# ishine/Test-time-adaptation-ASR-SUTA

Hardware: AMD Instinct MI355X
Metric: adapted utterances/sec (whole node) at 10 SUTA steps, w2v2-base; WER parity (higher is better)
Workload: dtype f32; 1 GPU; wav2vec2-base SUTA 10 steps on 128000-sample (8 s) utterances, 164 utterances per GPU per step, scripts/LS.sh flags; model=wav2vec2-base, global_batch=164, seq_len=399, n_samples=128000, suta_steps=10, parallelism=utterance-sharded x1

## Files before the change

test-time-adaptation-asr-suta_amd/csrc/common.h:

```cpp
#pragma once
#include <hip/hip_runtime.h>
#include <stdint.h>
#include <string>

#define SUTA_WAVE 64

typedef float f32x4 __attribute__((ext_vector_type(4)));
typedef float f32x16 __attribute__((ext_vector_type(16)));

__device__ __forceinline__ float gelu_f(float x) {
    return 0.5f * x * (1.0f + erff(x * 0.70710678118654752f));
}
__device__ __forceinline__ float dgelu_f(float x) {
    const float cdf = 0.5f * (1.0f + erff(x * 0.70710678118654752f));
    const float pdf = 0.39894228040143268f * __expf(-0.5f * x * x);
    return cdf + x * pdf;
}

__device__ __forceinline__ float erfc_t(float z, float t, float ez2) {
    float p = 0.17087277f;
    p = fmaf(p, t, -0.82215223f);
    p = fmaf(p, t, 1.48851587f);
    p = fmaf(p, t, -1.13520398f);
    p = fmaf(p, t, 0.27886807f);
    p = fmaf(p, t, -0.18628806f);
    p = fmaf(p, t, 0.09678418f);
    p = fmaf(p, t, 0.37409196f);
    p = fmaf(p, t, 1.00002368f);
    p = fmaf(p, t, -1.26551223f);
    return t * ez2 * __expf(p);
}
__device__ __forceinline__ float gelu_fast(float x) {
    const float z = fabsf(x) * 0.70710678118654752f;
    const float t = __builtin_amdgcn_rcpf(fmaf(0.5f, z, 1.0f));
    const float erfc = erfc_t(z, t, __expf(-z * z));
    return 0.5f * x * (x >= 0.f ? 2.0f - erfc : erfc);
}
__device__ __forceinline__ float dgelu_fast(float x) {
    const float z = fabsf(x) * 0.70710678118654752f;
    const float t = __builtin_amdgcn_rcpf(fmaf(0.5f, z, 1.0f));
    const float e = __expf(-z * z);
    const float erfc = erfc_t(z, t, e);
    const float cdf = 0.5f * (x >= 0.f ? 2.0f - erfc : erfc);
    return cdf + x * (0.39894228040143268f * e);
}

struct SutaSwitches {
    int latched;
    int fast_gelu;
    int flash_fwd_plane;
    int flash_bwd_plane;
    int flash_bf16_img;
    int conv_planes;
    int pre_bf16;
    int conv_z_bf16;
    int dy_planes;
    int conv_dx_planes;
    int fused_conv_ln;
    int flash_fwd_nw;
    int hbx;
    int splitk;
    int hbx_form;
    int ln_rpw;
    int hbx_dbg;
    int fused_delta;
    int hbx_t;
    int hbp_conv;
    int hbt4;
    int epi_fast;
    int loss_wide;
    int f32p;
    int sdpl_wide;
};
void suta_latch_switches();
void set_max_lds_once(const void* fn, size_t bytes, const char* name);
const SutaSwitches& suta_switches();

typedef float f32x2v __attribute__((ext_vector_type(2)));
__device__ __forceinline__ f32x2v phi_as2(f32x2v x, f32x2v& q) {
    const f32x2v z = __builtin_elementwise_abs(x) * 0.70710678118654752f;
    f32x2v p = z * 0.0000430638f + 0.0002765672f;
    p = p * z + 0.0001520143f;
    p = p * z + 0.0092705272f;
    p = p * z + 0.0422820123f;
    p = p * z + 0.0705230784f;
    p = p * z + 1.0f;
    p = p * p;
    p = p * p;
    p = p * p;
    p = p * p;
    q = f32x2v{__builtin_amdgcn_rcpf(p.x), __builtin_amdgcn_rcpf(p.y)};
    const f32x2v h = 0.5f * q;
    return f32x2v{x.x >= 0.f ? 1.0f - h.x : h.x, x.y >= 0.f ? 1.0f - h.y : h.y};
}
__device__ __forceinline__ f32x2v gelu2_bf16ep(f32x2v x) {
    f32x2v q;
    return x * phi_as2(x, q);
}
__device__ __forceinline__ f32x2v dgelu2_bf16ep(f32x2v x) {
    f32x2v q;
    const f32x2v cdf = phi_as2(x, q);
    const f32x2v a = x * x * (-0.5f * 1.4426950408889634f);
    const f32x2v e = f32x2v{__builtin_amdgcn_exp2f(a.x), __builtin_amdgcn_exp2f(a.y)};
    return cdf + (x * 0.39894228040143268f) * e;
}

__device__ __forceinline__ float wave_sum(float v) {
#pragma unroll
    for (int o = 32; o > 0; o >>= 1) v += __shfl_xor(v, o, 64);
    return v;
}
__device__ __forceinline__ double wave_sum_d(double v) {
#pragma unroll
    for (int o = 32; o > 0; o >>= 1) v += __shfl_xor(v, o, 64);
    return v;
}
__device__ __forceinline__ float wave_max(float v) {
#pragma unroll
    for (int o = 32; o > 0; o >>= 1) v = fmaxf(v, __shfl_xor(v, o, 64));
    return v;
}

enum {
    EPI_BIAS = 1,
    EPI_GELU = 2,
    EPI_RESID = 4,
    EPI_STORE_PRE = 8,
    EPI_DGELU = 16,
    EPI_ACCUM = 32,
    EPI_SMBWD = 64,
    EPI_ROWMASK = 128,
    EPI_DELTA = 256,
};

struct GemmParams {
    const float* A;
    const float* B;
    float* C;
    int M, N, K;
    long lda, ldb, ldc;
    int Z, zdiv;
    long sA0, sA1, sB0, sB1, sC0, sC1;
    int ta, tb;
    int segK, pad, Mvalid;
    int segB;
    long sBseg;
    const float* bias;
    long sBias0, sBias1;
    const float* R;
    long ldr, sR0, sR1;
    const float* aux;
    long ldaux, sAux0, sAux1;
    float* C2;
    long ldc2, sC20, sC21;
    const float* rowv;
    long sRow0, sRow1;
    const int* zrows;
    const int* zmvalid;
    float alpha;
    int epi;
    int splits, kchunk;
    float* ws;
    int va, vb;
    int mode;
    int order;
    const void* Ab;
    const void* Bb;
    long ldab, ldbb;
    void* Cb;
    long ldcb;
    long sCb1;
    int off32;
    int preb;
    int fgelu;
    const float* dlt_o;
    long ldo;
    float* delta;
    int dT, dNH;
};

void gemm_init(GemmParams& p);
bool gemm_hbx_t_selected(const GemmParams& p);
void gemm_launch(GemmParams p, hipStream_t st, float* ws, long ws_floats);
void gemm_set_variant(int tile, int nbuf);
void gemm_set_mode(int mode);
bool gemm_run_hb_class(const GemmParams& p, dim3 grid, hipStream_t st);
void launch_to_bf16(const float* src, long lds, long rows, int K, void* dst, hipStream_t st);
void launch_transpose_bf16(const float* src, long zs, int Z, int K, int N, void* dst, hipStream_t st,
                          void* dstn = nullptr);
int gemm_get_mode();
void gemm_census_enable(bool on);
std::string gemm_census_text();
bool gemm_census_is_on();
void gemm_census_time(const std::string& shape, double ms);
```

test-time-adaptation-asr-suta_amd/csrc/gemm.hip:

```cpp
#include "gemm_kernels.h"
#include <algorithm>
#include <cstdio>
#include <cstdlib>
#include <atomic>
#include <map>
#include <mutex>
#include <stdexcept>
#include <string>

namespace {

bool aligned16(const void* q) { return (reinterpret_cast<uintptr_t>(q) & 15) == 0; }

int g_force_tile = -1;
int g_nbuf = 3;
int g_mode = 0;

}

void gemm_set_variant(int tile, int nbuf) {
    g_force_tile = tile;
    g_nbuf = nbuf;
}

static std::mutex g_census_mu;
static std::map<std::string, long> g_census;
static std::atomic<bool> g_census_on{false};
static std::map<std::string, std::pair<double, long>> g_census_ms;

void gemm_census_enable(bool on) {
    std::lock_guard<std::mutex> lk(g_census_mu);
    g_census_on = on;
    g_census.clear();
    g_census_ms.clear();
}

bool gemm_census_is_on() { return g_census_on; }

void gemm_census_time(const std::string& shape, double ms) {
    std::lock_guard<std::mutex> lk(g_census_mu);
    auto& e = g_census_ms[shape];
    e.first += ms;
    e.second += 1;
}

std::string gemm_census_text() {
    std::lock_guard<std::mutex> lk(g_census_mu);
    std::string out;
    for (const auto& kv : g_census) out += kv.first + " " + std::to_string(kv.second) + "\n";
    for (const auto& kv : g_census_ms)
        out += "ms|" + kv.first + "|n=" + std::to_string(kv.second.second) + " " +
               std::to_string((long)(kv.second.first * 1000.0)) + "\n";
    return out;
}

static void census(const char* kernel, int BM, int BN, const GemmParams& p, int splits) {
    if (!g_census_on) return;
    char key[160], gkey[160], ekey[96];
    snprintf(key, sizeof key, "%s %dx%d z=%ld split=%d %s%s%s", kernel, BM, BN, (long)p.Z, splits, p.ta ? "T" : "N",
             p.tb ? "T" : "N", p.segK > 0 ? (p.segB ? " conv-seg" : " conv") : "");
    snprintf(gkey, sizeof gkey, "grid %s %dx%d gx=%d gy=%d z=%ld split=%d", kernel, BM, BN, (p.N + BN - 1) / BN,
             (p.M + BM - 1) / BM, (long)p.Z, splits);
    snprintf(ekey, sizeof ekey, "epi %s %dx%d %d", kernel, BM, BN, p.epi);
    std::lock_guard<std::mutex> lk(g_census_mu);
    ++g_census[key];
    ++g_census[gkey];
    ++g_census[ekey];
}

void gemm_set_mode(int mode) { g_mode = mode; }
int gemm_get_mode() { return g_mode; }

void gemm_init(GemmParams& p) {
    p = GemmParams{};
    p.Z = 1;
    p.zdiv = 1;
    p.alpha = 1.f;
    p.splits = 1;
    p.mode = g_mode;
}

static int choose_tile(long M, long N, long Z, long K, int mode) {
    struct Cand {
        int bm, bn;
        double eff;
    };
    static const Cand glds[4] = {{128, 128, 1.0}, {128, 64, 0.93}, {64, 128, 0.92}, {64, 64, 0.85}};
    static const Cand x6[4] = {{128, 128, 1.0}, {128, 64, 0.9}, {64, 128, 0.9}, {64, 64, 0.75}};
    const Cand* cands = mode == 0 ? glds : x6;
    int best = 0;
    double bt = 1e300;
    for (int c = 0; c < 4; ++c) {
        const long tiles = ((M + cands[c].bm - 1) / cands[c].bm) * ((N + cands[c].bn - 1) / cands[c].bn) * Z;
        const double area = (double)cands[c].bm * cands[c].bn;
        const double t = std::max((double)tiles, 256.0) * area / cands[c].eff;
        if (t < bt * 0.999) {
            bt = t;
            best = c;
        }
    }
    (void)K;
    return best;
}

static int choose_tile_bf16(long M, long N, long Z, bool big) {
    struct Cand {
        int id, bm, bn;
        double eff;
    };
    static const Cand c[5] = {{0, 128, 128, 1.0}, {4, 256, 128, 1.12}, {1, 128, 64, 0.85}, {2, 64, 128, 0.85},
                              {3, 64, 64, 0.6}};
    int best = 0;
    double bt = 1e300;
    for (int i = 0; i < 5; ++i) {
        if (c[i].id == 4 && !big) continue;
        const long tiles = ((M + c[i].bm - 1) / c[i].bm) * ((N + c[i].bn - 1) / c[i].bn) * Z;
        const double t = (double)((tiles + 511) / 512) * c[i].bm * c[i].bn / c[i].eff;
        if (t < bt * 0.999) {
            bt = t;
            best = c[i].id;
        }
    }
    return best;
}

static int choose_tile_hb(long M, long N, long Z) {
// ... 191 lines not shown
```

test-time-adaptation-asr-suta_amd/csrc/ops.h:

```cpp
#pragma once
#include "common.h"

void launch_wave_normalize(const float* x, float* y, int B, long N, const int* lens, hipStream_t st);

void launch_conv0(const float* x, long N, const float* W, const float* bias, long wstride, float* z, int B, int L0,
                  int C, int K, int S, hipStream_t st, void* zb = nullptr);

void launch_front_gn_fwd(const float* x, long N, const float* W, const float* bias, long wstride, int B, int L0, int C,
                         int K, int S, const float* g, const float* beta, float* mean, float* rstd, float* a,
                         double* dpart, const int* L0s, hipStream_t st);
void launch_front_gn_bwd(const float* x, long N, const float* W, const float* bias, long wstride, int B, int L0, int C,
                         int K, int S, const float* g, const float* beta, const float* mean, const float* rstd,
                         float* da, float* dgamma, float* dbeta, float* dW, long gstride, double* dpart, float* fpart,
                         const int* L0s, hipStream_t st);

void launch_layernorm_fwd(const float* x, const float* g, const float* beta, long pstride, int rows_per_utt,
                          float* y, float* xhat, float* rstd, int rows, int D, float eps, int gelu_out,
                          hipStream_t st, void* yb = nullptr, float* mean = nullptr, const void* xb = nullptr);
void launch_layernorm_bwd(const float* dy, const float* xhat, const float* rstd, const float* g, const float* beta,
                          long pstride, int rows_per_utt, int B, int D, int gelu_in, const float* post_aux,
                          const float* resid, float* dx, float* dgamma, float* dbeta, long gstride, float* part,
                          hipStream_t st, void* dxb = nullptr, const float* x = nullptr, const float* mean = nullptr,
                          const void* dyb = nullptr);

long layernorm_bwd_conv_part_floats(int B, int rows_per_utt, int D, int ktaps);
bool launch_layernorm_bwd_conv(const float* dy, const float* rstd, const float* g, const float* beta, long pstride,
                               int rows_per_utt, int B, int D, float* dx, float* dgamma, float* dbeta, float* dbias,
                               float* dw, long gstride, float* part, hipStream_t st, const float* x, const float* mean,
                               const float* xw, long xws, int xs, int ktaps, void* dxb = nullptr, int bf16_in = 0);
void launch_colsum(const float* x, int B, int rows, int C, float* out, long ostride, float* part, hipStream_t st);

struct AdapterW {
    const float *w1, *w1t, *w2, *w2t, *b1, *b2;
    int A, NA, Hp;
};
void launch_adapter_fwd(const float* x, const float* g, const float* beta, long pstride, int rows_per_utt, int B, int H,
                        const AdapterW& w, float eps, float* out, float* mean, float* rstd, hipStream_t st);
int adapter_padded_width(int A);
long adapter_part_floats(int B, int rows_per_utt, int H);
void launch_adapter_bwd(const float* x, const float* dout, const float* mean, const float* rstd, const float* g,
                        const float* beta, long pstride, int rows_per_utt, int B, int H, const AdapterW& w,
                        const int* tlen, float* dx, float* dgamma, float* dbeta, long gstride, float* part,
                        hipStream_t st, void* dxb = nullptr);

bool flash_dh_ok(int dh);
long flash_dq_scratch_floats(int B, int T, int NH, int dh);
bool flash_fwd_reads_plane(bool bf16, const void* qkvb, int H, int dh);
bool flash_bwd_reads_planes(bool bf16, const void* qkvb, const void* dctxb, int H, int dh);
bool launch_flash_fwd(const float* qkv, float* ctx, float* lse, int B, int T, int NH, int H, int dh, float scale,
                      const int* tlen, bool bf16, hipStream_t st, void* ctxb = nullptr, const void* qkvb = nullptr);
bool launch_flash_bwd(const float* qkv, const float* dctx, const float* lse, const float* delta, float* dqkv,
                      float* dqp, int B, int T, int NH, int H, int dh, float scale, const int* tlen, bool bf16,
                      hipStream_t st, void* dqkvb = nullptr, const void* qkvb = nullptr,
                      const void* dctxb = nullptr);
bool flash_wide_dh(int dh);
long flash_wide_dq_scratch_floats(int B, int T, int NH, int dh);
bool launch_flash_wide_fwd(const float* qkv, float* ctx, float* lse, int B, int T, int NH, int H, int dh, float scale,
                           const int* tlen, bool bf16, hipStream_t st, void* ctxb);
bool launch_flash_wide_bwd(const float* qkv, const float* dctx, const float* lse, const float* delta, float* dqkv,
                           float* dqp, int B, int T, int NH, int H, int dh, float scale, const int* tlen, bool bf16,
                           hipStream_t st, void* dqkvb);
bool launch_posconv(bool fwd, const float* x, const float* W, const float* bias, const float* R, float* C, float* C2,
                    int B, int T, int H, int G, int K, int pad, const int* tlen, hipStream_t st);
bool launch_posconv_bf16(bool fwd, const float* x, const void* Wt, const float* bias, const float* R, float* C,
                         float* C2, int B, int T, int H, int G, int K, int pad, const int* tlen, hipStream_t st);
void launch_softmax_rows(float* s, long nrows, int T, long ld, const int* tlen, long rows_per_utt, hipStream_t st);

void launch_attn_delta(const float* dO, const float* O, float* delta, int B, int T, int NH, int dh, hipStream_t st);

void launch_dgelu_mul(const float* g, const float* z, float* out, long n, hipStream_t st);

struct LossHP {
    float temp, em_coef, div_coef;
    int reweight, non_blank;
};
#define SUTA_MAX_VOCAB 1024
size_t suta_loss_scratch_floats(int B, long T, int V);
void launch_suta_loss(const float* logits, int B, int T, int V, LossHP hp, const int* tlen, float* dlogits, float* loss,
                      float* scratch, hipStream_t st);

enum { SDPL_KIND_NORMAL = 0, SDPL_KIND_DROP = 1, SDPL_KIND_SPACE = 2, SDPL_KIND_FAIL = 3 };
enum { SDPL_FLAG_LOOKUP = 1, SDPL_FLAG_INFEASIBLE = 2 };
struct SdplTable {
    const int* off;
    const int* ids;
    const int* kind;
    int space_id;
};
long sdpl_scratch_floats(int T, int V);
void launch_sdpl_loss(const float* logits, int B, int T, int V, float pl_coef, const int* tlen, float* dlogits,
                      float* loss, float* scratch, int* err, const SdplTable* tab, hipStream_t st);

void launch_argmax(const float* logits, long rows, int V, int* ids, hipStream_t st);

struct AdamRun {
    long start, len;
    int k;
};
#define SUTA_MAX_RUNS 32
#define ADAM_TAB 52
struct AdamArgs {
    int nruns;
    AdamRun runs[SUTA_MAX_RUNS];
    int blk0[SUTA_MAX_RUNS];
    float beta1, beta2, omb1, omb2, eps, lr_wd;
    int sgd;
    float step_size[5][5];
    float bc2_sqrt[5][5];
    const float* tab;
    const int* step;
};
void launch_broadcast(float* dst, const float* src, long n, int B, hipStream_t st);
void launch_step_advance(int* step, hipStream_t st);
void launch_adam(float* P, const float* G, float* M, float* V, long pstride, int B, const AdamArgs& a,
                 hipStream_t st);
```

test-time-adaptation-asr-suta_amd/csrc/ops.hip:

```cpp
#include "ops.h"
#include <algorithm>
#include <map>
#include <mutex>
#include <stdexcept>
#include <string>

namespace {

inline int cdiv(long a, long b) { return (int)((a + b - 1) / b); }

template <typename T>
__device__ __forceinline__ T block_sum(T v, T* red) {
    const int lane = threadIdx.x & 63, w = threadIdx.x >> 6;
#pragma unroll
    for (int o = 32; o > 0; o >>= 1) v += __shfl_xor(v, o, 64);
    __syncthreads();
    if (lane == 0) red[w] = v;
    __syncthreads();
    T s = red[0] + red[1] + red[2] + red[3];
    __syncthreads();
    return s;
}

__global__ __launch_bounds__(256) void wave_normalize_kernel(const float* __restrict__ x, float* __restrict__ y,
                                                             long N, const int* __restrict__ lens) {
    __shared__ double red[4];
    const float* xb = x + (long)blockIdx.x * N;
    float* yb = y + (long)blockIdx.x * N;
    const long n = lens ? lens[blockIdx.x] : N;
    double s = 0.0;
    for (long i = threadIdx.x; i < n; i += 256) s += xb[i];
    s = block_sum(s, red);
    const double mean = s / (double)n;
    double q = 0.0;
    for (long i = threadIdx.x; i < n; i += 256) {
        const double d = (double)xb[i] - mean;
        q += d * d;
    }
    q = block_sum(q, red);
    const float meanf = (float)mean;
    const float denom = (float)sqrt(q / (double)n + 1e-7);
    for (long i = threadIdx.x; i < N; i += 256) yb[i] = i < n ? (xb[i] - meanf) / denom : 0.f;
}

constexpr int C0_ROWS = 32;
__global__ __launch_bounds__(256) void conv0_kernel(const float* __restrict__ x, long N, const float* __restrict__ W,
                                                    const float* __restrict__ bias, long wstride,
                                                    float* __restrict__ z, int L0, int C, int K, int S) {
    __shared__ float xs[C0_ROWS * 16 + 16];
    const int b = blockIdx.y;
    const int t0 = blockIdx.x * C0_ROWS;
    const float* xb = x + (long)b * N;
    const float* Wb = W + (long)b * wstride;
    const float* bb = bias ? bias + (long)b * wstride : nullptr;
    const int nx = (C0_ROWS - 1) * S + K;
    for (int i = threadIdx.x; i < nx; i += 256) {
        const long gi = (long)t0 * S + i;
        xs[i] = gi < N ? xb[gi] : 0.f;
    }
    __syncthreads();
    const int rows = min(C0_ROWS, L0 - t0);
    float* zb = z + ((long)b * L0 + t0) * C;
    for (int c = threadIdx.x; c < C; c += 256) {
        float w[16];
#pragma unroll
        for (int k = 0; k < 16; ++k) w[k] = k < K ? Wb[(long)k * C + c] : 0.f;
        const float bv = bb ? bb[c] : 0.f;
        for (int r = 0; r < rows; ++r) {
            float acc = 0.f;
            for (int k = 0; k < K; ++k) acc = fmaf(xs[r * S + k], w[k], acc);
            zb[(long)r * C + c] = acc + bv;
        }
    }
}

typedef __bf16 lnbf16x4 __attribute__((ext_vector_type(4)));
__device__ __forceinline__ f32x4 load_bf16x4(const __bf16* src) {
    const lnbf16x4 b = *reinterpret_cast<const lnbf16x4*>(src);
    return f32x4{(float)b[0], (float)b[1], (float)b[2], (float)b[3]};
}
__device__ __forceinline__ void store_bf16x4(__bf16* dst, f32x4 v) {
    lnbf16x4 b;
#pragma unroll
    for (int e = 0; e < 4; ++e) b[e] = (__bf16)v[e];
    *reinterpret_cast<lnbf16x4*>(dst) = b;
}

constexpr int C0V_ROWS = 64;
// ... 716 lines not shown
    const int u = (L / ntile) % nutt;
    const int gi = L / (ntile * nutt);
    const int t0 = tile * WROWS;
    const int tl = tlen ? tlen[u] : T;
    const int w = threadIdx.x >> 6, lane = threadIdx.x & 63;
    const int r = lane & 15, g = lane >> 4;
    const float* xb = x + (long)u * T * H + gi * CG;
    const float* wg = W + (long)gi * K * CG * CG;

    const int nwin = (WROWS + K - 1) * (CG / 4);
    for (int it = threadIdx.x; it < nwin; it += NT) {
        const int row = it / (CG / 4), c4 = (it % (CG / 4)) * 4;
        const int t = t0 - pad + row;
        f32x4 v = {0.f, 0.f, 0.f, 0.f};
        if (t >= 0 && t < tl) v = *reinterpret_cast<const f32x4*>(xb + (long)t * H + c4);
        *reinterpret_cast<f32x4*>(win + row * XS + c4) = v;
    }
    f32x4 st[LPT];
    auto load_chunk = [&](int c) {
        const float* src = wg + (long)c * CHT * CG * CG;
#pragma unroll
        for (int n = 0; n < LPT; ++n) {
            const int it = threadIdx.x + n * NT;
            st[n] = it < CHUNK4 ? *reinterpret_cast<const f32x4*>(src + it * 4) : f32x4{0.f, 0.f, 0.f, 0.f};
        }
    };
    auto store_chunk = [&](int buf) {
        float* dst = wbuf + buf * (CHT * CG * WS);
#pragma unroll
        for (int n = 0; n < LPT; ++n) {
            const int it = threadIdx.x + n * NT;
            if (it < CHUNK4) {
                const int row = (it * 4) / CG, col = (it * 4) % CG;
                *reinterpret_cast<f32x4*>(dst + row * WS + col) = st[n];
            }
        }
    };
    f32x4 acc[NC];
#pragma unroll
    for (int nf = 0; nf < NC; ++nf) acc[nf] = f32x4{0.f, 0.f, 0.f, 0.f};
    const int nch = K / CHT;
    load_chunk(0);
    store_chunk(0);
    __syncthreads();
    const float* arow = win + (16 * w + r) * XS + g;
    for (int c = 0; c < nch; ++c) {
        if (c + 1 < nch) load_chunk(c + 1);
        const float* wb = wbuf + (c & 1) * (CHT * CG * WS) + g * WS + r;
#pragma unroll
        for (int qq = 0; qq < CHT; ++qq) {
            const float* ap = arow + (c * CHT + qq) * XS;
            const float* bp = wb + qq * CG * WS;
#pragma unroll
            for (int j = 0; j < CG / 4; ++j) {
                const float a = ap[4 * j];
                float b[NC];
#pragma unroll
                for (int nf = 0; nf < NC; ++nf) b[nf] = bp[4 * j * WS + 16 * nf];
#pragma unroll
                for (int nf = 0; nf < NC; ++nf) acc[nf] = __builtin_amdgcn_mfma_f32_16x16x4f32(a, b[nf], acc[nf], 0, 0, 0);
            }
        }
        if (c + 1 < nch) store_chunk((c + 1) & 1);
        __syncthreads();
    }
#pragma unroll
    for (int i = 0; i < 4; ++i) {
        const int t = t0 + 16 * w + 4 * g + i;
        if (t >= T) continue;
        const long o = ((long)u * T + t) * H + gi * CG;
#pragma unroll
        for (int nf = 0; nf < NC; ++nf) {
            const int co = 16 * nf + r;
            float v;
            if (FWD) {
                v = acc[nf][i] * 1.0f + bias[gi * CG + co];
                C2[o + co] = v;
                v = gelu_f(v) + R[o + co];
            } else {
                v = acc[nf][i] + R[o + co];
                if (tlen && t >= tl) v = 0.f;
            }
            C[o + co] = v;
        }
    }
}

constexpr int PCB_CHT = 4;
constexpr int PCB_RS = 72;
template <int WB, bool FWD>
__global__ __launch_bounds__(WB * 64, 1) void posconv_bf16_kernel(const float* __restrict__ x,
                                                                  const __bf16* __restrict__ Wt,
                                                                  const float* __restrict__ bias,
                                                                  const float* __restrict__ R, float* __restrict__ C,
                                                                  float* __restrict__ C2, int T, int H, int G, int K,
                                                                  int pad, const int* __restrict__ tlen, int ntile,
                                                                  int nutt) {
    constexpr int CG = 64, NT = WB * 64, WROWS = 32 * WB;
    constexpr int CHUNK = PCB_CHT * CG * CG / 8;
    constexpr int LPT = (CHUNK + NT - 1) / NT;
    extern __shared__ __attribute__((aligned(16))) __bf16 pcb_smem[];
    __bf16* win = pcb_smem;
    __bf16* wbuf = pcb_smem + (WROWS + K - 1) * PCB_RS;
    typedef __bf16 b8 __attribute__((ext_vector_type(8)));
    typedef __bf16 b4 __attribute__((ext_vector_type(4)));

    const int nb = gridDim.x;
    int L = blockIdx.x;
    if ((nb & 7) == 0) L = (L & 7) * (nb >> 3) + (L >> 3);
    const int tile = L % ntile;
    const int u = (L / ntile) % nutt;
    const int gi = L / (ntile * nutt);
    const int t0 = tile * WROWS;
    const int tl = tlen ? tlen[u] : T;
    const int w = threadIdx.x >> 6, lane = threadIdx.x & 63, l32 = lane & 31, h = lane >> 5;
    const float* xb = x + (long)u * T * H + gi * CG;
    const __bf16* wg = Wt + (long)gi * K * CG * CG;

    const int nwin = (WROWS + K - 1) * (CG / 4);
    for (int it = threadIdx.x; it < nwin; it += NT) {
        const int row = it / (CG / 4), c4 = (it % (CG / 4)) * 4;
        const int t = t0 - pad + row;
        f32x4 v = {0.f, 0.f, 0.f, 0.f};
        if (t >= 0 && t < tl) v = *reinterpret_cast<const f32x4*>(xb + (long)t * H + c4);
        b4 o;
#pragma unroll
        for (int e = 0; e < 4; ++e) o[e] = (__bf16)v[e];
        *reinterpret_cast<b4*>(win + row * PCB_RS + c4) = o;
    }
    b8 st[LPT];
    auto load_chunk = [&](int c) {
        const b8* src = reinterpret_cast<const b8*>(wg + (long)c * PCB_CHT * CG * CG);
#pragma unroll
        for (int n = 0; n < LPT; ++n) {
            const int it = threadIdx.x + n * NT;
            if (it < CHUNK) st[n] = src[it];
        }
    };
    auto store_chunk = [&](int buf) {
        __bf16* dst = wbuf + buf * (PCB_CHT * CG * PCB_RS);
#pragma unroll
        for (int n = 0; n < LPT; ++n) {
            const int it = threadIdx.x + n * NT;
            if (it < CHUNK) *reinterpret_cast<b8*>(dst + (it >> 3) * PCB_RS + (it & 7) * 8) = st[n];
        }
    };
    f32x16 acc[2];
#pragma unroll
    for (int nf = 0; nf < 2; ++nf)
#pragma unroll
        for (int v = 0; v < 16; ++v) acc[nf][v] = 0.f;
    const int nch = K / PCB_CHT;
    load_chunk(0);
    store_chunk(0);
    __syncthreads();
    const __bf16* arow = win + (32 * w + l32) * PCB_RS + 8 * h;
    for (int c = 0; c < nch; ++c) {
        if (c + 1 < nch) load_chunk(c + 1);
        const __bf16* wb = wbuf + (c & 1) * (PCB_CHT * CG * PCB_RS) + l32 * PCB_RS + 8 * h;
#pragma unroll
        for (int qq = 0; qq < PCB_CHT; ++qq) {
            const __bf16* ap = arow + (c * PCB_CHT + qq) * PCB_RS;
            const __bf16* bp = wb + qq * CG * PCB_RS;
#pragma unroll
            for (int kc = 0; kc < CG / 16; ++kc) {
                const b8 a = *reinterpret_cast<const b8*>(ap + 16 * kc);
// ... 886 lines not shown
            else                                                                                                 \
                hipLaunchKernelGGL((layernorm_bwd_conv_kernel<2, true, KT_, DB_, XB_>), grid, dim3(256), 0, st, dy,   \
                                   rstd, g, beta, pstride, rows_per_utt, dx, part, nchunk, crows, x, mean, xw, xws, \
                                   xs, reinterpret_cast<__bf16*>(dxb));                                          \
        } while (0)
        if (ktaps == 10) {
            if (dyb && xb) LBCB(10, true, true);
            else if (xb) LBCB(10, false, true);
            else return false;
        } else {
            if (dyb && xb) LBCB(0, true, true);
            else if (xb) LBCB(0, false, true);
            else return false;
        }
#undef LBCB
        const int nvec = 3 + ktaps;
        hipLaunchKernelGGL(chunk_reduce_conv, dim3(cdiv(D, 256), B, nvec), dim3(256), 0, st, part, nchunk, nvec, D,
                           dgamma, dbeta, dbias, dw, gstride);
        return true;
    }
#define LBC(GV_, KT_)                                                                                         \
    hipLaunchKernelGGL((layernorm_bwd_conv_kernel<2, GV_, KT_>), grid, dim3(256), 0, st, dy, rstd, g, beta, pstride, \
                       rows_per_utt, dx, part, nchunk, crows, x, mean, xw, xws, xs, reinterpret_cast<__bf16*>(dxb))
    if (ktaps == 10) {
        if (gv) LBC(true, 10);
        else LBC(false, 10);
    } else {
        if (gv) LBC(true, 0);
        else LBC(false, 0);
    }
#undef LBC
    const int nvec = 3 + ktaps;
    hipLaunchKernelGGL(chunk_reduce_conv, dim3(cdiv(D, 256), B, nvec), dim3(256), 0, st, part, nchunk, nvec, D, dgamma,
                       dbeta, dbias, dw, gstride);
    return true;
}

void launch_colsum(const float* x, int B, int rows, int C, float* out, long ostride, float* part, hipStream_t st) {
    const int nchunk = cdiv(rows, CS_ROWS);
    hipLaunchKernelGGL(colsum_partial, dim3(nchunk, B), dim3(256), 0, st, x, rows, C, part, nchunk);
    hipLaunchKernelGGL(chunk_reduce, dim3(cdiv(C, 256), B), dim3(256), 0, st, part, nchunk, 1, C, out, (float*)nullptr,
                       ostride);
}

void launch_softmax_rows(float* s, long nrows, int T, long ld, const int* tlen, long rows_per_utt, hipStream_t st) {
    dim3 grid((unsigned)((nrows + 3) / 4));
    if (T <= 256) hipLaunchKernelGGL(softmax_rows_kernel<4>, grid, dim3(256), 0, st, s, nrows, T, ld, tlen,
                                    rows_per_utt);
    else if (T <= 512) hipLaunchKernelGGL(softmax_rows_kernel<8>, grid, dim3(256), 0, st, s, nrows, T, ld, tlen,
                                    rows_per_utt);
    else if (T <= 1024) hipLaunchKernelGGL(softmax_rows_kernel<16>, grid, dim3(256), 0, st, s, nrows, T, ld, tlen,
                                    rows_per_utt);
    else hipLaunchKernelGGL(softmax_rows_kernel<32>, grid, dim3(256), 0, st, s, nrows, T, ld, tlen,
                                    rows_per_utt);
}

constexpr int PC_CHT = 2;
#define HIPCHK_OPS(x)                                                                        \
    do {                                                                                     \
        if ((x) != hipSuccess) throw std::runtime_error("hipFuncSetAttribute(posconv) failed"); \
    } while (0)

template <int CG, bool FWD>
static void posconv_go(int WB, dim3 grid, size_t lds, hipStream_t st, const float* x, const float* W,
                       const float* bias, const float* R, float* C, float* C2, int T, int H, int G, int K, int pad,
                       const int* tlen, int ntile, int B) {
#define PC(WB_)                                                                                                   \
    do {                                                                                                          \
        set_max_lds_once(reinterpret_cast<const void*>(&posconv_kernel<CG, WB_, PC_CHT, FWD>), 160 * 1024,       \
                         "posconv_kernel");                                                                       \
        hipLaunchKernelGGL((posconv_kernel<CG, WB_, PC_CHT, FWD>), grid, dim3(WB_ * 64), lds, st, x, W, bias, R, C, \
                           C2, T, H, G, K, pad, tlen, ntile, B);                                                  \
    } while (0)
    switch (WB) {
        case 4: PC(4); break;
        case 5: PC(5); break;
        case 6: PC(6); break;
        case 7: PC(7); break;
        default: PC(8); break;
    }
#undef PC
}

bool launch_posconv(bool fwd, const float* x, const float* W, const float* bias, const float* R, float* C, float* C2,
                    int B, int T, int H, int G, int K, int pad, const int* tlen, hipStream_t st) {
    const int CG = H / G;
    if ((CG != 48 && CG != 64) || K % PC_CHT || H % 4) return false;
    int WB = 8;
    long best = 1L << 40;
    for (int wb = 8; wb >= 4; --wb) {
        const long tiles = (T + 16 * wb - 1) / (16 * wb);
        const long waste = tiles * 16 * wb - T;
        if (waste < best) {
            best = waste;
            WB = wb;
        }
    }
    const int ntile = (T + 16 * WB - 1) / (16 * WB);
    const int XS = CG + 4, WS = (CG % 64 == 0) ? CG + 16 : CG;
    const size_t lds = ((size_t)(16 * WB + K - 1) * XS + 2 * PC_CHT * CG * WS) * sizeof(float);
    if (lds > 160 * 1024) return false;
    const dim3 grid((unsigned)((long)G * B * ntile));
    if (CG == 48) {
        if (fwd) posconv_go<48, true>(WB, grid, lds, st, x, W, bias, R, C, C2, T, H, G, K, pad, tlen, ntile, B);
        else posconv_go<48, false>(WB, grid, lds, st, x, W, bias, R, C, C2, T, H, G, K, pad, tlen, ntile, B);
    } else {
        if (fwd) posconv_go<64, true>(WB, grid, lds, st, x, W, bias, R, C, C2, T, H, G, K, pad, tlen, ntile, B);
        else posconv_go<64, false>(WB, grid, lds, st, x, W, bias, R, C, C2, T, H, G, K, pad, tlen, ntile, B);
    }
    return true;
}

template <bool FWD>
static void posconv_bf16_go(int WB, dim3 grid, size_t lds, hipStream_t st, const float* x, const __bf16* W,
                            const float* bias, const float* R, float* C, float* C2, int T, int H, int G, int K, int pad,
                            const int* tlen, int ntile, int B) {
#define PCB(WB_)                                                                                                  \
    do {                                                                                                          \
        set_max_lds_once(reinterpret_cast<const void*>(&posconv_bf16_kernel<WB_, FWD>), 160 * 1024,              \
                         "posconv_bf16_kernel");                                                                  \
        hipLaunchKernelGGL((posconv_bf16_kernel<WB_, FWD>), grid, dim3(WB_ * 64), lds, st, x, W, bias, R, C, C2, T, \
                           H, G, K, pad, tlen, ntile, B);                                                         \
    } while (0)
    switch (WB) {
        case 4: PCB(4); break;
        case 5: PCB(5); break;
        case 6: PCB(6); break;
        case 7: PCB(7); break;
        default: PCB(8); break;
    }
#undef PCB
}

bool launch_posconv_bf16(bool fwd, const float* x, const void* Wt, const float* bias, const float* R, float* C,
                         float* C2, int B, int T, int H, int G, int K, int pad, const int* tlen, hipStream_t st) {
    if (H / G != 64 || H % G || K % PCB_CHT || !Wt) return false;
    int WB = 8;
    long best = 1L << 40;
    for (int wb = 8; wb >= 4; --wb) {
        const long tiles = (T + 32 * wb - 1) / (32 * wb);
        const long waste = tiles * 32 * wb - T;
        if (waste < best) {
            best = waste;
            WB = wb;
        }
    }
    const int ntile = (T + 32 * WB - 1) / (32 * WB);
    const size_t lds = ((size_t)(32 * WB + K - 1) * PCB_RS + 2 * PCB_CHT * 64 * PCB_RS) * sizeof(__bf16);
    if (lds > 160 * 1024) return false;
    const dim3 grid((unsigned)((long)G * B * ntile));
    const __bf16* W = reinterpret_cast<const __bf16*>(Wt);
    if (fwd) posconv_bf16_go<true>(WB, grid, lds, st, x, W, bias, R, C, C2, T, H, G, K, pad, tlen, ntile, B);
    else posconv_bf16_go<false>(WB, grid, lds, st, x, W, bias, R, C, C2, T, H, G, K, pad, tlen, ntile, B);
    return true;
}

void launch_dgelu_mul(const float* g, const float* z, float* out, long n, hipStream_t st) {
    hipLaunchKernelGGL(dgelu_mul_kernel, dim3(ew_grid(n)), dim3(256), 0, st, g, z, out, n);
}

void launch_suta_loss(const float* logits, int B, int T, int V, LossHP hp, const int* tlen, float* dlogits, float* loss,
                      float* scratch, hipStream_t st) {
    if (V < 1 || V > SUTA_MAX_VOCAB) throw std::runtime_error("suta loss: vocab_size outside [1, 1024]");
    if (V <= 64 && !suta_switches().loss_wide) {
        hipLaunchKernelGGL(suta_loss_kernel, dim3(B), dim3(256), 0, st, logits, T, V, hp, dlogits, loss, scratch, tlen);
        return;
    }
    double* rowd = reinterpret_cast<double*>(scratch);
    double* utt = rowd + (size_t)B * T * LW_ROW;
    double* cls = utt + (size_t)B * LW_UTT;
    const long rows = (long)B * T;
    const dim3 rgrid((unsigned)((rows + 3) / 4));
    const double temp = hp.temp;
    hipLaunchKernelGGL(loss_wide_rows_kernel, rgrid, dim3(256), 0, st, logits, T, V, rows, temp, dlogits, rowd, tlen);
    hipLaunchKernelGGL(loss_wide_utt_kernel, dim3(B), dim3(256), 0, st, T, hp.reweight, rowd, utt, tlen);
    hipLaunchKernelGGL(loss_wide_cols_kernel, dim3((V + 63) / 64, B), dim3(256), 0, st, logits, T, V, temp, rowd, cls,
                       tlen);
    hipLaunchKernelGGL(loss_wide_finish_kernel, dim3(B), dim3(256), 0, st, T, V, hp, cls, utt, loss, tlen);
    hipLaunchKernelGGL(loss_wide_grad_kernel, rgrid, dim3(256), 0, st, logits, T, V, rows, hp, rowd, utt, cls, dlogits,
                       tlen);
}

size_t suta_loss_scratch_floats(int B, long T, int V) {
    const size_t narrow = (size_t)B * T * 66 + 64;
    const size_t wide = 2 * ((size_t)B * T * LW_ROW + (size_t)B * LW_UTT + (size_t)B * V * LW_CLS) + 64;
// ... 14 lines not shown
}

void launch_broadcast(float* dst, const float* src, long n, int B, hipStream_t st) {
    if (n % 4) throw std::runtime_error("broadcast length not a multiple of 4");
    const long n4 = n / 4;
    hipLaunchKernelGGL(broadcast_kernel, dim3((unsigned)((n4 + 255) / 256), B), dim3(256), 0, st,
                       reinterpret_cast<f32x4*>(dst), reinterpret_cast<const f32x4*>(src), n4);
}

__global__ void step_advance_kernel(int* step) { *step += 1; }

void launch_step_advance(int* step, hipStream_t st) {
    hipLaunchKernelGGL(step_advance_kernel, dim3(1), dim3(1), 0, st, step);
}

void launch_adam(float* P, const float* G, float* M, float* V, long pstride, int B, const AdamArgs& a,
                 hipStream_t st) {
    AdamArgs aa = a;
    long nblk = 0;
    for (int r = 0; r < a.nruns; ++r) {
        if (a.runs[r].start % 4) throw std::runtime_error("adam run start not 16-B aligned");
        if (a.runs[r].k < 1 || a.runs[r].k > 5) throw std::runtime_error("adam multiplicity outside [1, 5]");
        aa.blk0[r] = (int)nblk;
        nblk += ((a.runs[r].len + 3) / 4 + 256 * ADAM_GPT - 1) / (256 * ADAM_GPT);
    }
    if (nblk == 0) return;
    if (pstride % 4) throw std::runtime_error("adam slot stride not a multiple of 4");
    hipLaunchKernelGGL(adam_kernel, dim3((unsigned)nblk, B), dim3(256), 0, st, P, G, M, V, pstride, aa);
}

void set_max_lds_once(const void* fn, size_t bytes, const char* name) {
    static std::mutex mu;
    static std::map<const void*, size_t> done;
    std::lock_guard<std::mutex> lk(mu);
    auto it = done.find(fn);
    if (it != done.end() && it->second >= bytes) return;
    if (hipFuncSetAttribute(fn, hipFuncAttributeMaxDynamicSharedMemorySize, (int)bytes) != hipSuccess)
        throw std::runtime_error(std::string("hipFuncSetAttribute(") + name + ") failed");
    done[fn] = bytes;
}

static thread_local SutaSwitches g_switches{};

void suta_latch_switches() {
    auto on = [](const char* name) {
        const char* ev = std::getenv(name);
        return (ev && atoi(ev) == 0) ? 0 : 1;
    };
    SutaSwitches s{};
    s.fast_gelu = on("SUTA_FAST_GELU");
    s.flash_fwd_plane = on("SUTA_FLASH_FWD_PLANE");
    s.flash_bwd_plane = on("SUTA_FLASH_BWD_PLANE");
    s.flash_bf16_img = on("SUTA_FLASH_BF16_IMG");
    s.conv_planes = on("SUTA_CONV_PLANES");
    s.pre_bf16 = on("SUTA_PRE_BF16");
    s.conv_z_bf16 = on("SUTA_CONV_Z_BF16");
    s.dy_planes = on("SUTA_DY_PLANES");
    s.conv_dx_planes = on("SUTA_CONV_DX_PLANES");
    s.fused_conv_ln = on("SUTA_FUSED_CONV_LN");
    const char* hbx = std::getenv("SUTA_HBX");
    s.hbx = hbx ? atoi(hbx) : 1;
    s.splitk = on("SUTA_SPLITK");
    const char* hbxt = std::getenv("SUTA_HBX_T");
    s.hbx_t = hbxt ? std::min(2, std::max(0, atoi(hbxt))) : 2;
    s.fused_delta = on("SUTA_FUSED_DELTA");
    const char* lrpw = std::getenv("SUTA_LN_RPW");
    s.ln_rpw = lrpw ? atoi(lrpw) : 2;
    const char* hform = std::getenv("SUTA_HBX_FORM");
    s.hbx_form = hform ? atoi(hform) : 4;
    const char* ht4 = std::getenv("SUTA_HBT4");
    s.hbt4 = ht4 ? atoi(ht4) : 1;
    const char* hdbg = std::getenv("SUTA_HBX_DBG");
    s.hbx_dbg = hdbg ? atoi(hdbg) : 0;
    const char* fnw = std::getenv("SUTA_FLASH_FWD_NW");
    s.flash_fwd_nw = (fnw && atoi(fnw) == 8) ? 8 : 4;
    s.epi_fast = on("SUTA_EPI_FAST");
    s.hbp_conv = on("SUTA_HBP_CONV");
    const char* lw = std::getenv("SUTA_LOSS_WIDE");
    s.loss_wide = (lw && atoi(lw) != 0) ? 1 : 0;
    const char* f32p = std::getenv("SUTA_F32P");
    s.f32p = f32p ? std::min(2, std::max(0, atoi(f32p))) : 1;
    const char* sw = std::getenv("SUTA_SDPL_WIDE");
    s.sdpl_wide = (sw && atoi(sw) != 0) ? 1 : 0;
    s.latched = 1;
    g_switches = s;
}

const SutaSwitches& suta_switches() {
    if (!g_switches.latched) suta_latch_switches();
    return g_switches;
}

static bool fast_gelu_on() { return suta_switches().fast_gelu != 0; }
template <int MODE, typename... Args>
static void launch_conv0_gn(dim3 grid, hipStream_t st, int K, int S, Args... args) {
    if (K == 10 && S == 5 && fast_gelu_on())
        hipLaunchKernelGGL((conv0_gn_kernel<MODE, 10, 5, true>), grid, dim3(256), 0, st, args...);
    else if (K == 10 && S == 5)
        hipLaunchKernelGGL((conv0_gn_kernel<MODE, 10, 5>), grid, dim3(256), 0, st, args...);
    else
        hipLaunchKernelGGL((conv0_gn_kernel<MODE, 0, 0>), grid, dim3(256), 0, st, args...);
}

void launch_front_gn_fwd(const float* x, long N, const float* W, const float* bias, long wstride, int B, int L0, int C,
                         int K, int S, const float* g, const float* beta, float* mean, float* rstd, float* a,
                         double* dpart, const int* L0s, hipStream_t st) {
    const int nchunk = cdiv(L0, F0_ROWS);
    launch_conv0_gn<0>(dim3(nchunk, B), st, K, S, x, N, W, bias, wstride, L0, C, K, S,
                       (const float*)nullptr, (const float*)nullptr, (const float*)nullptr, (const float*)nullptr,
                       (float*)nullptr, (const float*)nullptr, dpart, (float*)nullptr, nchunk, L0s);
    hipLaunchKernelGGL(col_stats_final, dim3(cdiv(C, 256), B), dim3(256), 0, st, dpart, nchunk, L0, C, 1e-5f, mean,
                       rstd, L0s);
    launch_conv0_gn<1>(dim3(nchunk, B), st, K, S, x, N, W, bias, wstride, L0, C, K, S,
                       mean, rstd, g, beta, a, (const float*)nullptr, (double*)nullptr, (float*)nullptr, nchunk, L0s);
}

void launch_front_gn_bwd(const float* x, long N, const float* W, const float* bias, long wstride, int B, int L0, int C,
                         int K, int S, const float* g, const float* beta, const float* mean, const float* rstd,
                         float* da, float* dgamma, float* dbeta, float* dW, long gstride, double* dpart, float* fpart,
                         const int* L0s, hipStream_t st) {
    const int nchunk = cdiv(L0, F0_ROWS);
    launch_conv0_gn<2>(dim3(nchunk, B), st, K, S, x, N, W, bias, wstride, L0, C, K, S,
                       mean, rstd, g, beta, da, (const float*)nullptr, dpart, (float*)nullptr, nchunk, L0s);
    float* coef = reinterpret_cast<float*>(dpart + (long)B * nchunk * 2 * C);
    hipLaunchKernelGGL(gn_bwd_final, dim3(cdiv(C, 256), B), dim3(256), 0, st, dpart, nchunk, C, dgamma, dbeta, gstride,
                       coef);
    launch_conv0_gn<3>(dim3(nchunk, B), st, K, S, x, N, W, bias, wstride, L0, C, K, S,
                       mean, rstd, g, beta, da, coef, (double*)nullptr, fpart, nchunk, L0s);
    hipLaunchKernelGGL(conv0_dw_reduce, dim3(cdiv((long)K * C, 256), B), dim3(256), 0, st, fpart, nchunk, K * C, dW,
                       gstride);
}

void launch_attn_delta(const float* dO, const float* O, float* delta, int B, int T, int NH, int dh, hipStream_t st) {
    const long items = (long)B * T * NH;
    const long vec = items * (dh / 4);
    const dim3 grid((unsigned)((vec + 255) / 256));
    const f32x4* a = reinterpret_cast<const f32x4*>(dO);
    const f32x4* c = reinterpret_cast<const f32x4*>(O);
    switch (dh) {
        case 16: hipLaunchKernelGGL(attn_delta_kernel<4>, grid, dim3(256), 0, st, a, c, delta, items, T, NH); return;
        case 32: hipLaunchKernelGGL(attn_delta_kernel<8>, grid, dim3(256), 0, st, a, c, delta, items, T, NH); return;
        case 64: hipLaunchKernelGGL(attn_delta_kernel<16>, grid, dim3(256), 0, st, a, c, delta, items, T, NH); return;
        case 128: hipLaunchKernelGGL(attn_delta_kernel<32>, grid, dim3(256), 0, st, a, c, delta, items, T, NH); return;
        default:
            if (dh % 4 == 0 && dh <= 128 && (reinterpret_cast<uintptr_t>(dO) & 15) == 0 &&
                (reinterpret_cast<uintptr_t>(O) & 15) == 0) {
                hipLaunchKernelGGL(attn_delta_pad32_kernel, dim3((unsigned)((items * 32 + 255) / 256)), dim3(256), 0, st,
                                   a, c, delta, items, T, NH, dh / 4);
                return;
            }
            hipLaunchKernelGGL(attn_delta_scalar, dim3((unsigned)((items + 255) / 256)), dim3(256), 0, st, dO, O, delta,
                               items, T, NH, dh);
    }
}
```

Baseline: 39.35 utt/s.

## Add span-based positional conv kernel with cost-model planner choosing tile or span

Adds a new positional-convolution kernel in which each 8-wave block covers a span of many 16-frame fragments, with several fragments per wave. This amortizes staging of the weight chunks across more output frames. A planner header models LDS occupancy, rounds over CUs and MFMA throughput, then picks between the existing tile kernel (any WB 4..8) and span variants. The span path is on by default through an env switch. The risks are reduced occupancy from large LDS windows and a cost model whose constants may not match the real hardware.

```diff
diff --git a/test-time-adaptation-asr-suta_amd/csrc/common.h b/test-time-adaptation-asr-suta_amd/csrc/common.h
--- a/test-time-adaptation-asr-suta_amd/csrc/common.h
+++ b/test-time-adaptation-asr-suta_amd/csrc/common.h
@@ -71,6 +71,8 @@
     int loss_wide;
     int f32p;
     int sdpl_wide;
+    int posconv_span;
+    int posconv_wb;
 };
 void suta_latch_switches();
 void set_max_lds_once(const void* fn, size_t bytes, const char* name);
@@ -193,3 +195,4 @@
 std::string gemm_census_text();
 bool gemm_census_is_on();
 void gemm_census_time(const std::string& shape, double ms);
+void gemm_census_count(const std::string& key);
diff --git a/test-time-adaptation-asr-suta_amd/csrc/gemm.hip b/test-time-adaptation-asr-suta_amd/csrc/gemm.hip
--- a/test-time-adaptation-asr-suta_amd/csrc/gemm.hip
+++ b/test-time-adaptation-asr-suta_amd/csrc/gemm.hip
@@ -42,6 +42,12 @@
     auto& e = g_census_ms[shape];
     e.first += ms;
     e.second += 1;
+}
+
+void gemm_census_count(const std::string& key) {
+    if (!g_census_on) return;
+    std::lock_guard<std::mutex> lk(g_census_mu);
+    ++g_census[key];
 }
 
 std::string gemm_census_text() {
diff --git a/test-time-adaptation-asr-suta_amd/csrc/ops.h b/test-time-adaptation-asr-suta_amd/csrc/ops.h
--- a/test-time-adaptation-asr-suta_amd/csrc/ops.h
+++ b/test-time-adaptation-asr-suta_amd/csrc/ops.h
@@ -1,5 +1,6 @@
 #pragma once
 #include "common.h"
+#include "posconv_plan.h"
 
 void launch_wave_normalize(const float* x, float* y, int B, long N, const int* lens, hipStream_t st);
 
@@ -62,6 +63,7 @@
                            hipStream_t st, void* dqkvb);
 bool launch_posconv(bool fwd, const float* x, const float* W, const float* bias, const float* R, float* C, float* C2,
                     int B, int T, int H, int G, int K, int pad, const int* tlen, hipStream_t st);
+bool posconv_plan_for(int B, int T, int H, int G, int K, PosconvPlan* out);
 bool launch_posconv_bf16(bool fwd, const float* x, const void* Wt, const float* bias, const float* R, float* C,
                          float* C2, int B, int T, int H, int G, int K, int pad, const int* tlen, hipStream_t st);
 void launch_softmax_rows(float* s, long nrows, int T, long ld, const int* tlen, long rows_per_utt, hipStream_t st);
diff --git a/test-time-adaptation-asr-suta_amd/csrc/ops.hip b/test-time-adaptation-asr-suta_amd/csrc/ops.hip
--- a/test-time-adaptation-asr-suta_amd/csrc/ops.hip
+++ b/test-time-adaptation-asr-suta_amd/csrc/ops.hip
@@ -4,6 +4,7 @@
 #include <mutex>
 #include <stdexcept>
 #include <string>
+#include <type_traits>
 
 namespace {
 
@@ -886,6 +887,133 @@
                 if (tlen && t >= tl) v = 0.f;
             }
             C[o + co] = v;
+        }
+    }
+}
+
+template <int CG, int FPW, int CHT, bool FWD>
+__global__ __launch_bounds__(512, 1) void posconv_span_kernel(const float* __restrict__ x,
+                                                              const float* __restrict__ W,
+                                                              const float* __restrict__ bias,
+                                                              const float* __restrict__ R, float* __restrict__ C,
+                                                              float* __restrict__ C2, int T, int H, int G, int K,
+                                                              int pad, const int* __restrict__ tlen, int nspan,
+                                                              int nutt, int F) {
+    constexpr int NW = 8, NT = NW * 64, NC = CG / 16, XS = PcLayout<CG>::XS, WS = PcLayout<CG>::WS;
+    constexpr int CHUNK4 = CHT * CG * CG / 4;
+    constexpr int LPT = (CHUNK4 + NT - 1) / NT;
+    extern __shared__ __attribute__((aligned(16))) float pc_smem[];
+    float* win = pc_smem;
+    float* wbuf = pc_smem + (16 * F + K - 1) * XS;
+
+    const int nb = gridDim.x;
+    int L = blockIdx.x;
+    if ((nb & 7) == 0) L = (L & 7) * (nb >> 3) + (L >> 3);
+    const int span = L % nspan;
+    const int u = (L / nspan) % nutt;
+    const int gi = L / (nspan * nutt);
+    const int nf_here = min(F, (T + 15) / 16 - span * F);
+    const int t0 = span * F * 16;
+    const int tl = tlen ? tlen[u] : T;
+    const int w = threadIdx.x >> 6, lane = threadIdx.x & 63;
+    const int r = lane & 15, g = lane >> 4;
+    const int nown = nf_here > w ? (nf_here - w + NW - 1) / NW : 0;
+    const float* xb = x + (long)u * T * H + gi * CG;
+    const float* wg = W + (long)gi * K * CG * CG;
+
+    const int nwin = (16 * nf_here + K - 1) * (CG / 4);
+    for (int it = threadIdx.x; it < nwin; it += NT) {
+        const int row = it / (CG / 4), c4 = (it % (CG / 4)) * 4;
+        const int t = t0 - pad + row;
+        f32x4 v = {0.f, 0.f, 0.f, 0.f};
+        if (t >= 0 && t < tl) v = *reinterpret_cast<const f32x4*>(xb + (long)t * H + c4);
+        *reinterpret_cast<f32x4*>(win + row * XS + c4) = v;
+    }
+    f32x4 st[LPT];
+    auto load_chunk = [&](int c) {
+        const float* src = wg + (long)c * CHT * CG * CG;
+#pragma unroll
+        for (int n = 0; n < LPT; ++n) {
+            const int it = threadIdx.x + n * NT;
+            st[n] = it < CHUNK4 ? *reinterpret_cast<const f32x4*>(src + it * 4) : f32x4{0.f, 0.f, 0.f, 0.f};
+        }
+    };
+    auto store_chunk = [&](int buf) {
+        float* dst = wbuf + buf * (CHT * CG * WS);
+#pragma unroll
+        for (int n = 0; n < LPT; ++n) {
+            const int it = threadIdx.x + n * NT;
+            if (it < CHUNK4) {
+                const int row = (it * 4) / CG, col = (it * 4) % CG;
+                *reinterpret_cast<f32x4*>(dst + row * WS + col) = st[n];
+            }
+        }
+    };
+    f32x4 acc[FPW][NC];
+#pragma unroll
+    for (int i = 0; i < FPW; ++i)
+#pragma unroll
+        for (int nf = 0; nf < NC; ++nf) acc[i][nf] = f32x4{0.f, 0.f, 0.f, 0.f};
+    const int nch = K / CHT;
+    load_chunk(0);
+    store_chunk(0);
+    __syncthreads();
+    const float* arow = win + (16 * w + r) * XS + g;
+    auto taps = [&](auto n_) {
+        constexpr int N = decltype(n_)::value;
+        for (int c = 0; c < nch; ++c) {
+            if (c + 1 < nch) load_chunk(c + 1);
+            const float* wb = wbuf + (c & 1) * (CHT * CG * WS) + g * WS + r;
+#pragma unroll
+            for (int qq = 0; qq < CHT; ++qq) {
+                const float* ap = arow + (c * CHT + qq) * XS;
+                const float* bp = wb + qq * CG * WS;
+#pragma unroll
+                for (int j = 0; j < CG / 4; ++j) {
+                    float a[N > 0 ? N : 1];
+#pragma unroll
+                    for (int i = 0; i < N; ++i) a[i] = ap[i * (16 * NW * XS) + 4 * j];
+                    float b[NC];
+#pragma unroll
+                    for (int nf = 0; nf < NC; ++nf) b[nf] = bp[4 * j * WS + 16 * nf];
+#pragma unroll
+                    for (int i = 0; i < N; ++i)
+#pragma unroll
+                        for (int nf = 0; nf < NC; ++nf)
+                            acc[i][nf] = __builtin_amdgcn_mfma_f32_16x16x4f32(a[i], b[nf], acc[i][nf], 0, 0, 0);
+                }
+            }
+            if (c + 1 < nch) store_chunk((c + 1) & 1);
+            __syncthreads();
+        }
+    };
+    if (nown >= FPW) taps(std::integral_constant<int, FPW>{});
+    else if (FPW > 3 && nown == 3) taps(std::integral_constant<int, (FPW > 3 ? 3 : 0)>{});
+    else if (FPW > 2 && nown == 2) taps(std::integral_constant<int, (FPW > 2 ? 2 : 0)>{});
+    else if (FPW > 1 && nown == 1) taps(std::integral_constant<int, (FPW > 1 ? 1 : 0)>{});
+    else taps(std::integral_constant<int, 0>{});
+#pragma unroll
+    for (int i = 0; i < FPW; ++i) {
+        if (i >= nown) break;
+#pragma unroll
+        for (int ii = 0; ii < 4; ++ii) {
+            const int t = t0 + 16 * (w + NW * i) + 4 * g + ii;
+            if (t >= T) continue;
+            const long o = ((long)u * T + t) * H + gi * CG;
+#pragma unroll
+            for (int nf = 0; nf < NC; ++nf) {
+                const int co = 16 * nf + r;
+                float v;
+                if (FWD) {
+                    v = acc[i][nf][ii] * 1.0f + bias[gi * CG + co];
+                    C2[o + co] = v;
+                    v = gelu_f(v) + R[o + co];
+                } else {
+                    v = acc[i][nf][ii] + R[o + co];
+                    if (tlen && t >= tl) v = 0.f;
+                }
+                C[o + co] = v;
+            }
         }
     }
 }
@@ -1938,25 +2066,77 @@
 #undef PC
 }
 
+template <int CG, bool FWD>
+static void posconv_span_go(const PosconvPlan& pl, hipStream_t st, const float* x, const float* W, const float* bias,
+                            const float* R, float* C, float* C2, int T, int H, int G, int K, int pad, const int* tlen,
+                            int B) {
+#define PCS(FPW_)                                                                                                  \
+    do {                                                                                                           \
+        set_max_lds_once(reinterpret_cast<const void*>(&posconv_span_kernel<CG, FPW_, PC_CHT, FWD>), PC_LDS_MAX,   \
+                         "posconv_span_kernel");                                                                   \
+        hipLaunchKernelGGL((posconv_span_kernel<CG, FPW_, PC_CHT, FWD>), dim3((unsigned)pl.grid), dim3(pl.threads), \
+                           pl.lds, st, x, W, bias, R, C, C2, T, H, G, K, pad, tlen, pl.nblk, B, pl.F);             \
+    } while (0)
+    constexpr int FPW_MAX = CG == 48 ? PC_SPAN_FPW_MAX : 2;
+    if (pl.FPW > FPW_MAX) throw std::runtime_error("posconv span: fragments per wave beyond the built forms");
+    switch (pl.FPW) {
+        case 1: PCS(1); break;
+        case 2: PCS(2); break;
+        case 3: PCS((FPW_MAX >= 3 ? 3 : 1)); break;
+        default: PCS((FPW_MAX >= 4 ? 4 : 1)); break;
+    }
+#undef PCS
+}
+
+static int device_cus() {
+    static std::mutex mu;
+    static std::map<int, int> cus;
+    int dev = 0;
+    if (hipGetDevice(&dev) != hipSuccess) throw std::runtime_error("hipGetDevice failed");
+    std::lock_guard<std::mutex> lk(mu);
+    auto it = cus.find(dev);
+    if (it != cus.end()) return it->second;
+    hipDeviceProp_t prop;
+    if (hipGetDeviceProperties(&prop, dev) != hipSuccess) throw std::runtime_error("hipGetDeviceProperties failed");
+    return cus[dev] = std::max(1, prop.multiProcessorCount);
+}
+
+bool posconv_plan_for(int B, int T, int H, int G, int K, PosconvPlan* out) {
+    const int CG = H / G;
+    if ((CG != 48 && CG != 64) || K % PC_CHT || H % 4) return false;
+    const SutaSwitches& sw = suta_switches();
+    PosconvPlan pl = posconv_plan(T, CG, K, PC_CHT, G, B, device_cus(), sw.posconv_span, sw.posconv_wb);
+    if (pl.span && pl.FPW > (CG == 48 ? PC_SPAN_FPW_MAX : 2))
+        pl = posconv_span_plan(T, CG, K, PC_CHT, G, B, device_cus(), 8 * (CG == 48 ? PC_SPAN_FPW_MAX : 2));
+    if (pl.lds > (size_t)PC_LDS_MAX) return false;
+    *out = pl;
+    return true;
+}
+
 bool launch_posconv(bool fwd, const float* x, const float* W, const float* bias, const float* R, float* C, float* C2,
                     int B, int T, int H, int G, int K, int pad, const int* tlen, hipStream_t st) {
+    PosconvPlan pl;
+    if (!posconv_plan_for(B, T, H, G, K, &pl)) return false;
     const int CG = H / G;
-    if ((CG != 48 && CG != 64) || K % PC_CHT || H % 4) return false;
-    int WB = 8;
-    long best = 1L << 40;
-    for (int wb = 8; wb >= 4; --wb) {
-        const long tiles = (T + 16 * wb - 1) / (16 * wb);
-        const long waste = tiles * 16 * wb - T;
-        if (waste < best) {
-            best = waste;
-            WB = wb;
-        }
-    }
-    const int ntile = (T + 16 * WB - 1) / (16 * WB);
-    const int XS = CG + 4, WS = (CG % 64 == 0) ? CG + 16 : CG;
-    const size_t lds = ((size_t)(16 * WB + K - 1) * XS + 2 * PC_CHT * CG * WS) * sizeof(float);
-    if (lds > 160 * 1024) return false;
-    const dim3 grid((unsigned)((long)G * B * ntile));
+    if (gemm_census_is_on()) {
+        char key[96];
+        if (pl.span) snprintf(key, sizeof key, "posconv span CG=%d F=%d FPW=%d spans=%d", CG, pl.F, pl.FPW, pl.nblk);
+        else snprintf(key, sizeof key, "posconv tile CG=%d WB=%d tiles=%d", CG, pl.WB, pl.nblk);
+        gemm_census_count(key);
+    }
+    if (pl.span) {
+        if (CG == 48) {
+            if (fwd) posconv_span_go<48, true>(pl, st, x, W, bias, R, C, C2, T, H, G, K, pad, tlen, B);
+            else posconv_span_go<48, false>(pl, st, x, W, bias, R, C, C2, T, H, G, K, pad, tlen, B);
+        } else {
+            if (fwd) posconv_span_go<64, true>(pl, st, x, W, bias, R, C, C2, T, H, G, K, pad, tlen, B);
+            else posconv_span_go<64, false>(pl, st, x, W, bias, R, C, C2, T, H, G, K, pad, tlen, B);
+        }
+        return true;
+    }
+    const int WB = pl.WB, ntile = pl.nblk;
+    const size_t lds = pl.lds;
+    const dim3 grid((unsigned)pl.grid);
     if (CG == 48) {
         if (fwd) posconv_go<48, true>(WB, grid, lds, st, x, W, bias, R, C, C2, T, H, G, K, pad, tlen, ntile, B);
         else posconv_go<48, false>(WB, grid, lds, st, x, W, bias, R, C, C2, T, H, G, K, pad, tlen, ntile, B);
@@ -2137,6 +2317,11 @@
     s.f32p = f32p ? std::min(2, std::max(0, atoi(f32p))) : 1;
     const char* sw = std::getenv("SUTA_SDPL_WIDE");
     s.sdpl_wide = (sw && atoi(sw) != 0) ? 1 : 0;
+    const char* pcs = std::getenv("SUTA_POSCONV_SPAN");
+    s.posconv_span = pcs ? std::max(0, atoi(pcs)) : 1;
+    const char* pcw = std::getenv("SUTA_POSCONV_WB");
+    s.posconv_wb = pcw ? atoi(pcw) : 0;
+    if (s.posconv_wb < 4 || s.posconv_wb > 8) s.posconv_wb = 0;
     s.latched = 1;
     g_switches = s;
 }
diff --git a/test-time-adaptation-asr-suta_amd/csrc/posconv_plan.h b/test-time-adaptation-asr-suta_amd/csrc/posconv_plan.h
--- /dev/null
+++ b/test-time-adaptation-asr-suta_amd/csrc/posconv_plan.h
@@ -0,0 +1,118 @@
+#pragma once
+#include <cstddef>
+
+constexpr int PC_LDS_MAX = 160 * 1024;
+constexpr int PC_LDS_GRANULE = 1280;
+constexpr int PC_SPAN_WAVES = 8;
+constexpr int PC_SPAN_FPW_MAX = 4;
+constexpr double PC_WAVE_LATENCY_UNITS = 1.5;
+constexpr double PC_STAGE_UNITS_PER_FRAG = 0.045;
+
+struct PosconvPlan {
+    int span;
+    int WB;
+    int F;
+    int FPW;
+    int nblk;
+    long grid;
+    int threads;
+    size_t lds;
+    int per_cu;
+    long rounds;
+    double units;
+    double cost;
+};
+
+inline size_t posconv_lds_bytes(int CG, int K, int CHT, int frags) {
+    const int XS = CG + 4, WS = (CG % 64 == 0) ? CG + 16 : CG;
+    return ((size_t)(16 * frags + K - 1) * XS + (size_t)2 * CHT * CG * WS) * sizeof(float);
+}
+
+inline int posconv_span_simd_frags(int F) {
+    auto wave = [F](int w) { return F > w ? (F - w + PC_SPAN_WAVES - 1) / PC_SPAN_WAVES : 0; };
+    return wave(0) + wave(4);
+}
+
+inline void posconv_rate(PosconvPlan& p, int G, int B, int CUs) {
+    const int alloc = (int)((p.lds + PC_LDS_GRANULE - 1) / PC_LDS_GRANULE) * PC_LDS_GRANULE;
+    int per_cu = PC_LDS_MAX / alloc;
+    const int by_waves = 32 / (p.threads / 64);
+    if (per_cu > by_waves) per_cu = by_waves;
+    if (per_cu < 1) per_cu = 1;
+    p.grid = (long)G * B * p.nblk;
+    if ((long)per_cu > (p.grid + CUs - 1) / CUs) per_cu = (int)((p.grid + CUs - 1) / CUs);
+    p.per_cu = per_cu;
+    const long slots = (long)CUs * per_cu;
+    const long rounds = (p.grid + slots - 1) / slots;
+    const int simd = p.span ? posconv_span_simd_frags(p.F) : (p.WB + 3) / 4;
+    const double mfma = (double)per_cu * simd, wave = p.FPW + PC_WAVE_LATENCY_UNITS;
+    p.rounds = rounds;
+    p.units = (double)rounds * mfma;
+    p.cost = (double)rounds * ((mfma > wave ? mfma : wave) + PC_STAGE_UNITS_PER_FRAG * per_cu * p.F);
+}
+
+inline PosconvPlan posconv_tile_plan(int T, int CG, int K, int CHT, int G, int B, int CUs, int WB) {
+    PosconvPlan p{};
+    p.span = 0;
+    p.WB = p.F = WB;
+    p.FPW = 1;
+    p.nblk = (T + 16 * WB - 1) / (16 * WB);
+    p.threads = 64 * WB;
+    p.lds = posconv_lds_bytes(CG, K, CHT, WB);
+    posconv_rate(p, G, B, CUs);
+    return p;
+}
+
+inline PosconvPlan posconv_span_plan(int T, int CG, int K, int CHT, int G, int B, int CUs, int F) {
+    PosconvPlan p{};
+    const int nfrag = (T + 15) / 16;
+    p.span = 1;
+    p.WB = PC_SPAN_WAVES;
+    p.F = F;
+    p.FPW = (F + PC_SPAN_WAVES - 1) / PC_SPAN_WAVES;
+    p.nblk = (nfrag + F - 1) / F;
+    p.threads = 64 * PC_SPAN_WAVES;
+    p.lds = posconv_lds_bytes(CG, K, CHT, F);
+    posconv_rate(p, G, B, CUs);
+    return p;
+}
+
+inline int posconv_span_max(int CG, int K, int CHT) {
+    int F = 0;
+    while (F < PC_SPAN_WAVES * PC_SPAN_FPW_MAX && posconv_lds_bytes(CG, K, CHT, F + 1) <= (size_t)PC_LDS_MAX) ++F;
+    return F;
+}
+
+inline int posconv_legacy_wb(int T) {
+    int WB = 8;
+    long best = 1L << 40;
+    for (int wb = 8; wb >= 4; --wb) {
+        const long tiles = (T + 16 * wb - 1) / (16 * wb);
+        const long waste = tiles * 16 * wb - T;
+        if (waste < best) {
+            best = waste;
+            WB = wb;
+        }
+    }
+    return WB;
+}
+
+inline PosconvPlan posconv_plan(int T, int CG, int K, int CHT, int G, int B, int CUs, int span_switch = 1,
+                                int wb_override = 0) {
+    if (wb_override >= 4 && wb_override <= 8) return posconv_tile_plan(T, CG, K, CHT, G, B, CUs, wb_override);
+    PosconvPlan best = posconv_tile_plan(T, CG, K, CHT, G, B, CUs, posconv_legacy_wb(T));
+    if (span_switch == 0) return best;
+    const int fmax = posconv_span_max(CG, K, CHT);
+    if (span_switch >= 2) {
+        if (fmax < 1) return best;
+        return posconv_span_plan(T, CG, K, CHT, G, B, CUs, span_switch < fmax ? span_switch : fmax);
+    }
+    auto consider = [&best](const PosconvPlan& p) {
+        if (p.lds > (size_t)PC_LDS_MAX) return;
+        if (best.lds > (size_t)PC_LDS_MAX || p.cost < best.cost || (p.cost == best.cost && p.lds < best.lds)) best = p;
+    };
+    for (int wb = 4; wb <= 8; ++wb) consider(posconv_tile_plan(T, CG, K, CHT, G, B, CUs, wb));
+    const int nfrag = (T + 15) / 16;
+    for (int F = 1; F <= fmax && F <= nfrag; ++F) consider(posconv_span_plan(T, CG, K, CHT, G, B, CUs, F));
+    return best;
+}
```

After: 39.57 utt/s (median of 6 runs). About the same (+0.6%).
